# TropComplique/single-shot-detector

Hardware: AMD Instinct MI355X
Metric: images/sec at 896x640, MobileNet-v1 RetinaNet (whole hot path incl. decode + per-class NMS) (higher is better)
Workload: dtype f32

## Files before the change

include/ssd_hip.h:

```cpp
#ifndef SSD_HIP_H
#define SSD_HIP_H

#include <stddef.h>
#include <stdint.h>

#ifdef __cplusplus
extern "C" {
#endif

#define SSD_OK 0
#define SSD_ERR_INVALID (-1)
#define SSD_ERR_HIP (-2)
#define SSD_ERR_STATE (-3)
#define SSD_ERR_WEIGHT (-4)

#define SSD_ACT_NONE 0
#define SSD_ACT_RELU 1
#define SSD_ACT_RELU6 2

#define SSD_BACKBONE_MOBILENET 0
#define SSD_BACKBONE_SHUFFLENET 1

#define SSD_PRECISION_F32 0
#define SSD_PRECISION_F16X3 1
// ... 33 lines not shown
int ssd_forward_records(ssd_handle *h, const uint8_t *images_dev, int32_t B, int32_t H, int32_t W,
                        void *records_dev, void *stream);
int ssd_forward_host(ssd_handle *h, const uint8_t *images_host, int32_t B, int32_t H, int32_t W,
                     void *records, void *stream);

int ssd_network_shape(ssd_handle *h, int32_t height, int32_t width, int32_t *net_hw_out );
int ssd_forward_mixed(ssd_handle *h, const uint8_t *images_dev, int32_t B, const int32_t *hw_host, const int64_t *offsets_host,
                      void *records_dev, void *stream);
int ssd_forward_mixed_host(ssd_handle *h, const uint8_t *const *frames_host, int32_t B, const int32_t *hw_host, void *records,
                           void *stream);

int ssd_detect_host(ssd_handle *h, const uint8_t *image_host, int32_t H, int32_t W, float score_threshold,
                    void *record, float *boxes_out, int32_t *labels_out, float *scores_out, int32_t capacity,
                    int32_t *n_out, void *stream);

int ssd_get_tensor(ssd_handle *h, const char *name, float *host_dst, int64_t capacity_floats,
                   int32_t *dims_out);

int ssd_get_tensor_dev(ssd_handle *h, const char *name, float *dst_dev, int64_t capacity_floats,
                       int32_t *dims_out, void *stream);

int ssd_plan_cache_stats(ssd_handle *h, int64_t *out8);
int ssd_plan_cache_clear(ssd_handle *h);

int ssd_profile_enable(ssd_handle *h, int32_t on);
int ssd_profile_read(ssd_handle *h, int32_t cls, double *total_ms, int64_t *launches,
                     double *flops, double *bytes);
int ssd_profile_reset(ssd_handle *h);


int32_t ssd_num_anchors(int32_t H, int32_t W);
int ssd_anchors(int32_t H, int32_t W, float *anchors_host );
int64_t ssd_anchors_ex(int32_t H, int32_t W, int32_t n_levels, const int32_t *strides, const double *scales,
                       int32_t n_mult, const double *multipliers, int32_t n_ratios, const double *ratios,
                       float *anchors_host, int64_t capacity_rows);

int ssd_conv2d(const float *in_dev, int32_t B, int32_t H, int32_t W, int32_t Cin,
               const float *w_host , int32_t k, int32_t Cout,
               int32_t stride, int32_t pad_beg, int32_t OH, int32_t OW,
               const float *bn_mean_host, const float *bn_sf_host, const float *bn_beta_host,
               const float *bias_host, const float *up_dev, int32_t act, float *out_dev,
               void *stream);

int ssd_conv2d_f16x3(const float *in_dev, int32_t B, int32_t H, int32_t W, int32_t Cin,
                     const float *w_host , int32_t k, int32_t Cout,
                     int32_t stride, int32_t pad_beg, int32_t OH, int32_t OW,
// ... 241 lines not shown
```

single-shot-detector_amd/_lib.py:

```python
import ctypes
import os
import subprocess

_HERE = os.path.dirname(os.path.abspath(__file__))
_CSRC = os.path.join(_HERE, "csrc")
_SOURCES = ["abi.hip", "weights.hip", "plan.hip", "stages.hip", "igemm.hip", "igemm_lat.hip", "igemm16.hip", "logit_screen.hip", "dwpw_stream.hip", "sn_pw.hip", "front.hip",
            "elementwise.hip", "postprocess.hip", "loss.hip", "augment.hip", "update.hip", "train_head.hip", "wgrad.hip", "train_backbone.hip", "train_shufflenet.hip",
            "train_first_f32.hip", "train_norms.hip", "train_hist.hip", "train_reduce.hip"]
_LIB_PATH = os.path.join(_CSRC, "libssd_hip.so")
_DIAG_PATH = os.path.join(_CSRC, "libssd_hip_diag.so")
_lib = None
_diag = False

HIPCC_FLAGS = ["--offload-arch=gfx950", "-O3", "-ffp-contract=off", "-fPIC", "-shared", "-std=c++17"]


class SsdError(RuntimeError):
    """A non-zero return code from libssd_hip.so (message from ssd_last_error())."""


def lib_path():
    return _LIB_PATH


# ... 106 lines not shown
class SsdBnLevel(ctypes.Structure):
    _fields_ = [("rows", ctypes.c_int64)] + [(n, ctypes.c_void_p) for n in (
        "x", "dy", "out", "gamma", "beta", "moving_mean", "moving_variance", "mean", "var", "invstd", "dgamma", "dbeta")]


SIGNATURES = {
    "ssd_create": (ctypes.c_int, [ctypes.POINTER(SsdConfig), ctypes.POINTER(_vp)]),
    "ssd_destroy": (None, [_vp]),
    "ssd_last_error": (ctypes.c_char_p, []),
    "ssd_load_weight": (ctypes.c_int, [_vp, ctypes.c_char_p, _f, ctypes.POINTER(ctypes.c_int64), _i]),
    "ssd_finalize": (ctypes.c_int, [_vp]),
    "ssd_forward": (ctypes.c_int, [_vp, _vp, _i, _i, _i, _vp, _vp, _vp, _vp, _vp]),
    "ssd_record_words": (ctypes.c_int32, [_vp]),
    "ssd_forward_records": (ctypes.c_int, [_vp, _vp, _i, _i, _i, _vp, _vp]),
    "ssd_forward_host": (ctypes.c_int, [_vp, _vp, _i, _i, _i, _vp, _vp]),
    "ssd_network_shape": (ctypes.c_int, [_vp, _i, _i, _i32p]),
    "ssd_forward_mixed": (ctypes.c_int, [_vp, _vp, _i, _i32p, ctypes.POINTER(ctypes.c_int64), _vp, _vp]),
    "ssd_forward_mixed_host": (ctypes.c_int, [_vp, ctypes.POINTER(ctypes.c_void_p), _i, _i32p, _vp, _vp]),
    "ssd_detect_host": (ctypes.c_int, [_vp, _vp, _i, _i, ctypes.c_float, _vp, _vp, _vp, _vp, _i, _i32p, _vp]),
    "ssd_get_tensor": (ctypes.c_int, [_vp, ctypes.c_char_p, _f, ctypes.c_int64, _i32p]),
    "ssd_get_tensor_dev": (ctypes.c_int, [_vp, ctypes.c_char_p, _vp, ctypes.c_int64, _i32p, _vp]),
    "ssd_plan_cache_stats": (ctypes.c_int, [_vp, ctypes.POINTER(ctypes.c_int64)]),
    "ssd_plan_cache_clear": (ctypes.c_int, [_vp]),
    "ssd_profile_enable": (ctypes.c_int, [_vp, _i]),
    "ssd_profile_read": (ctypes.c_int, [_vp, _i, ctypes.POINTER(ctypes.c_double),
                                        ctypes.POINTER(ctypes.c_int64),
                                        ctypes.POINTER(ctypes.c_double),
                                        ctypes.POINTER(ctypes.c_double)]),
    "ssd_profile_reset": (ctypes.c_int, [_vp]),
    "ssd_num_anchors": (ctypes.c_int32, [_i, _i]),
    "ssd_anchors": (ctypes.c_int, [_i, _i, _f]),
    "ssd_anchors_ex": (ctypes.c_int64, [_i, _i, _i, _i32p, ctypes.POINTER(ctypes.c_double), _i, ctypes.POINTER(ctypes.c_double),
                                        _i, ctypes.POINTER(ctypes.c_double), _f, ctypes.c_int64]),
    "ssd_conv2d": (ctypes.c_int, [_vp, _i, _i, _i, _i, _f, _i, _i, _i, _i, _i, _i, _f, _f, _f, _f,
                                  _vp, _i, _vp, _vp]),
    "ssd_conv2d_f16x3": (ctypes.c_int, [_vp, _i, _i, _i, _i, _f, _i, _i, _i, _i, _i, _i, _f, _f, _f, _f,
                                        _vp, _i, _vp, _vp]),
    "ssd_set_option": (ctypes.c_int, [_vp, ctypes.c_char_p, _i]),
    "ssd_get_option": (ctypes.c_int, [_vp, ctypes.c_char_p, _i32p]),
    "ssd_set_precision": (ctypes.c_int, [_vp, _i]),
    "ssd_get_precision": (ctypes.c_int, [_vp]),
    "ssd_status": (ctypes.c_int, [_vp, _i32p]),
    "ssd_depthwise3x3": (ctypes.c_int, [_vp, _i, _i, _i, _i, _f, _i, _i, _i, _i, _f, _f, _f, _i,
                                        _vp, _vp]),
    "ssd_dw_pw": (ctypes.c_int, [_vp, _i, _i, _i, _i, _f, _i, _f, _f, _f, _i, _f, _i, _f, _f, _f, _i, _vp, _vp]),
    "ssd_first_conv": (ctypes.c_int, [_vp, _i, _i, _i, _f, _i, _f, _f, _f, _i, _vp, _vp]),
# ... 119 lines not shown
```

single-shot-detector_amd/csrc/abi.hip:

```cpp
#include "host.h"

#include <algorithm>
#include <cmath>
#include <cstdio>
#include <cstring>

static thread_local std::string g_err;
int ssd_fail(int code, const std::string &msg) { g_err = msg; return code; }
extern "C" const char *ssd_last_error(void) { return g_err.c_str(); }

static Options g_opts;
static std::mutex g_opts_mu;
static const char *const OPT_NAMES[OPT_COUNT] = {"streams", "h2d_chunks", "front_fuse", "fuse_dw", "backbone_split", "event_fence", "plan_cache_mb",
                                                 "igemm_tile", "igemm16", "igemm_96", "igemm_lat", "igemm_deep64", "lateral_split", "fpn_group", "fpn_p7_group",
                                                 "fpn_early_lat", "nsub", "nms_fast_max", "first_conv_px", "debug_sync", "logits_screen",
                                                 "hist_scheme"};
int ssd_opt_index(const char *key)
{
    for (int i = 0; i < OPT_COUNT; ++i)
        if (key && !strcmp(key, OPT_NAMES[i])) return i;
    return -1;
}
int ssd_opt(const ssd_handle *h, int key, int dflt)
{
    if (h && h->opts.v[key] != SSD_OPT_UNSET) return h->opts.v[key];
    const int g = g_opts.v[key];
    return g != SSD_OPT_UNSET ? g : dflt;
}
unsigned ssd_sync_event_flags(const ssd_handle *h)
{
    return hipEventDisableTiming | (ssd_opt(h, OPT_EVENT_FENCE, 0) ? 0u : (unsigned)hipEventDisableSystemFence);
}
int nms_fast_max(const ssd_handle *h)
{
    const int v = ssd_opt(h, OPT_NMS_FAST_MAX, -1);
    return v < 0 ? 0 : (v == 0 ? -1 : v);
}

// ... 492 lines not shown
        else HIPCHK(hipMemcpyAsync(dst_dev + done, r.dev, (size_t)rows * r.C * sizeof(float), hipMemcpyDeviceToDevice, (hipStream_t)stream));
        done += rows * r.C;
        Btot += r.B;
        dims[1] = r.H; dims[2] = r.W; dims[3] = r.C;
    }
    dims[0] = Btot;
    return SSD_OK;
}

extern "C" int ssd_plan_cache_stats(ssd_handle *h, int64_t *out)
{
    if (!h || !out) return ssd_fail(SSD_ERR_INVALID, "ssd_plan_cache_stats: null argument");
    std::lock_guard<std::mutex> g(h->mu);
    HIPCHK(hipSetDevice(h->cfg.device));
    size_t total = 0;
    for (const PlanSet *ps : h->cache) total += ps->bytes;
    out[0] = (int64_t)h->cache.size();
    out[1] = (int64_t)total;
    out[2] = (int64_t)plan_cache_limit_bytes(h);
    out[3] = h->cache_hits; out[4] = h->cache_misses; out[5] = h->cache_evictions;
    out[6] = h->cur ? h->cur->key.netH : 0;
    out[7] = h->cur ? h->cur->key.netW : 0;
    return SSD_OK;
}

extern "C" int ssd_plan_cache_clear(ssd_handle *h)
{
    if (!h) return ssd_fail(SSD_ERR_INVALID, "ssd_plan_cache_clear: null handle");
    std::lock_guard<std::mutex> g(h->mu);
    HIPCHK(hipSetDevice(h->cfg.device));
    HIPCHK(hipDeviceSynchronize());
    h->cache_evictions += (long long)h->cache.size();
    free_plans(h);
    h->n_rec_ok = 0;
    return SSD_OK;
}

extern "C" int ssd_profile_enable(ssd_handle *h, int32_t on)
{
    if (!h) return ssd_fail(SSD_ERR_INVALID, "null handle");
    std::lock_guard<std::mutex> g(h->mu);
    h->profiling = on != 0;
    return SSD_OK;
}

static int drain_events(ssd_handle *h)
// ... 59 lines not shown
```

single-shot-detector_amd/csrc/host.h:

```cpp
#pragma once
#include "../../include/ssd_hip.h"
#include "ssd_internal.h"

#include <climits>
#include <functional>
#include <map>
#include <mutex>
#include <string>
#include <vector>

int ssd_fail(int code, const std::string &msg);
#define HIPCHK(expr)                                                                         \
    do {                                                                                     \
        hipError_t e_ = (expr);                                                              \
        if (e_ != hipSuccess)                                                                \
            return ssd_fail(SSD_ERR_HIP, std::string(#expr) + ": " + hipGetErrorString(e_)); \
    } while (0)
#define SSDCHK(expr)                                                                         \
    do {                                                                                     \
        int r_ = (expr);                                                                     \
        if (r_ != SSD_OK) return r_;                                                         \
    } while (0)

enum SsdOpt {
    OPT_STREAMS = 0,
    OPT_H2D_CHUNKS,
    OPT_FRONT_FUSE,
    OPT_FUSE_DW,
    OPT_BACKBONE_SPLIT,
    OPT_EVENT_FENCE,
    OPT_PLAN_CACHE_MB,
    OPT_IGEMM_TILE,
    OPT_IGEMM16,
    OPT_IGEMM_96,
    OPT_IGEMM_LAT,
    OPT_IGEMM_DEEP64,
    OPT_LATERAL_SPLIT,
    OPT_FPN_GROUP,
    OPT_FPN_P7_GROUP,
    OPT_FPN_EARLY_LAT,
    OPT_NSUB,
    OPT_NMS_FAST_MAX,
    OPT_FIRST_CONV_PX,
    OPT_DEBUG_SYNC,
    OPT_LOGITS_SCREEN,
    OPT_HIST_SCHEME,
    OPT_COUNT
};
#define SSD_OPT_UNSET INT_MIN
struct Options { int v[OPT_COUNT]; Options() { for (int &x : v) x = SSD_OPT_UNSET; } };
int ssd_opt(const struct ssd_handle *h, int key, int dflt);
int ssd_opt_index(const char *key);
unsigned ssd_sync_event_flags(const struct ssd_handle *h);

struct Tensor {
    std::vector<int64_t> shape;
    std::vector<float> data;
};

struct DevPool {
    std::vector<void *> ptrs;
    size_t bytes = 0;
    int alloc(void **out, size_t nbytes)
    {
        HIPCHK(hipMalloc(out, nbytes + 256));
        ptrs.push_back(*out);
        bytes += nbytes + 256;
        return SSD_OK;
// ... 106 lines not shown
int nms_fast_max(const struct ssd_handle *h);

struct ResizeDims { int nh, nw, ph, pw; float box_scaler[4]; };
ResizeDims resize_dims(int height, int width, int min_dimension, int divisor);
extern const int A_STRIDES[5];
extern const int MB_STRIDE[13];

struct Retained { const float *dev; int B, H, W, C, Cp; bool permuted; int fmt = 0;
                  int split = 0;  };

struct EvPair { hipEvent_t a, b; int cls; int fwd; };

struct Plan {
    int B = 0, img0 = 0, N = 0;
    DevPool pool;
    std::vector<Op> ops;
    PostArgs post;
    std::map<std::string, Retained> retained;
    hipStream_t s_aux = nullptr;
    hipStream_t s_bb[2] = {nullptr, nullptr};
    hipEvent_t ev_join = nullptr, ev_begin = nullptr;
    bool need_begin = false;
    bool screened = false, logits_whole = true;
    Op logits_dense;
};

struct SrcGeom { int srcH = 0, srcW = 0, nh = 0, nw = 0; float box_scaler[4] = {1, 1, 1, 1}; };

struct MixedCall { MixedGeom geom; float scaler[SSD_MIXED_MAX][2]; };

struct PlanKey {
    int B = 0, netH = 0, netW = 0, ident = 0, nsub = 0;
    bool operator==(const PlanKey &o) const { return B == o.B && netH == o.netH && netW == o.netW && ident == o.ident && nsub == o.nsub; }
};
struct PlanSet {
    PlanKey key;
    std::vector<Plan *> plans;
    size_t bytes = 0;
    unsigned long long last_use = 0;
};

struct ssd_handle {
    ssd_config cfg;
    std::mutex mu;
    Options opts;
    std::map<std::string, Tensor> vars;
// ... 52 lines not shown
```

single-shot-detector_amd/csrc/logit_screen.hip:

```cpp
#include "ssd_internal.h"
#include <type_traits>

typedef float v16f __attribute__((ext_vector_type(16)));
typedef float v4f __attribute__((ext_vector_type(4)));
typedef unsigned v4u __attribute__((ext_vector_type(4)));
typedef _Float16 v8h __attribute__((ext_vector_type(8)));
typedef short v2s __attribute__((ext_vector_type(2)));
typedef __attribute__((address_space(3))) void *lds_ptr_t;

#define SCREEN_STAGE_BYTES ((256 + 128) * 128)
#define SCREEN_STAGES 3

__device__ __forceinline__ unsigned f16_up_bits(float x)
{
    if (!(x >= 0.0f)) return 0x7e00u;
    if (x == 0.0f) return 0u;
    const _Float16 h = (_Float16)x;
    unsigned b = (unsigned)__builtin_bit_cast(unsigned short, h);
    if ((float)h < x) b += 1u;
    return b < 0x0400u ? 0x0400u : b;
}

__global__ __launch_bounds__(256) void logit_convert_kernel(const float *__restrict__ x, unsigned short *__restrict__ x16, long long n8)
{
// ... 3 lines not shown
        o[0] = f16_up_bits(a[0]) | (f16_up_bits(a[1]) << 16);
        o[1] = f16_up_bits(a[2]) | (f16_up_bits(a[3]) << 16);
        o[2] = f16_up_bits(b[0]) | (f16_up_bits(b[1]) << 16);
        o[3] = f16_up_bits(b[2]) | (f16_up_bits(b[3]) << 16);
        *(v4u *)(x16 + i * 8) = o;
    }
}

__device__ __forceinline__ ScreenLevel screen_level_of_tile(const ScreenArgs &a, int tile_m)
{
    ScreenLevel L = a.lv[0];
#pragma unroll
    for (int i = 1; i < SCREEN_MAX_LEVELS; ++i)
        if (i < a.nlevels && tile_m >= a.lv[i].tile_begin) L = a.lv[i];
    return L;
}
__device__ __forceinline__ ScreenLevel screen_level_of_row(const ScreenArgs &a, int r)
{
    ScreenLevel L = a.lv[0];
#pragma unroll
    for (int i = 1; i < SCREEN_MAX_LEVELS; ++i)
        if (i < a.nlevels && r >= a.lv[i].row_begin) L = a.lv[i];
    return L;
}

__device__ __forceinline__ v8h screen_operand(v4u f, unsigned sgn)
{
    v4u o;
#pragma unroll
    for (int d = 0; d < 4; ++d) {
        const v2s h = __builtin_bit_cast(v2s, f[d] ^ sgn);
        o[d] = __builtin_bit_cast(unsigned, __builtin_elementwise_max(h, v2s{0, 0}));
    }
    return __builtin_bit_cast(v8h, o);
}

__global__ __launch_bounds__(256, 1) void logit_screen_kernel(const ScreenArgs a)
{
    constexpr int BM = 256;
    constexpr int A_BYTES = BM * 128;
    constexpr int STAGE = SCREEN_STAGE_BYTES;
    constexpr int NSTAGE = SCREEN_STAGES;
    extern __shared__ __attribute__((aligned(16))) unsigned char lds[];

    const int tid = threadIdx.x, lane = tid & 63;
    const int wave = __builtin_amdgcn_readfirstlane(tid >> 6);
// ... 158 lines not shown
        for (int j = 0; j < 4; ++j)
#pragma unroll
            for (int r = 0; r < 16; ++r) mine[(r * 4 + j) * 64 + lane] = acc[i][j][r];
        __syncthreads();
        const int rbase = m0 + wave_m * 128 + i * 32;
#pragma unroll 1
        for (int r = wave_n * 8; r < wave_n * 8 + 8; ++r) {
            const int rowl = rbase + (r & 3) + 8 * (r >> 2) + 4 * (lane >> 5);
#pragma unroll
            for (int j = 0; j < 4; ++j) {
                const float Pv = Pp[(r * 4 + j) * 64 + lane], Nv = Np[(r * 4 + j) * 64 + lane];
                const float t1 = Pv * 1.001953125f, t2 = Nv * 0.998046875f;
                const float U = ((t1 - t2) + cst[j]) + 3.814697265625e-06f * ((Pv + Nv) + __builtin_fabsf(cst[j]));
                const bool flag = colok[j] && rowl < M && !(U < lo);
                const unsigned long long mask = __ballot(flag);
                if (mask != 0ull && lane < 8) {
                    const unsigned byte = (unsigned)(mask >> (8 * lane)) & 0xffu;
                    const int row = rbase + (r & 3) + 8 * (r >> 2) + 4 * (lane >> 2);
                    const int col8 = tile_n * 128 + j * 32 + (lane & 3) * 8;
                    if (byte && row < M && col8 < a.Cout) {
                        const int b = row / P, p = row - b * P;
                        const unsigned oct = (unsigned)((out_off + (long long)b * bstride + (long long)p * rstride + col8) >> 3);
                        atomicOr(a.bits + (oct >> 5), 1u << (oct & 31));
                    }
                }
            }
        }
        __syncthreads();
    };
    pass(std::integral_constant<int, 0>{});
    pass(std::integral_constant<int, 1>{});
    pass(std::integral_constant<int, 2>{});
    pass(std::integral_constant<int, 3>{});
}

__global__ __launch_bounds__(256) void logit_compact_kernel(const ScreenArgs a, long long nwords)
{
    __shared__ int lcnt[SCREEN_MAX_OCT], lbase[SCREEN_MAX_OCT];
    __shared__ unsigned short slot[256 * 32];
    const int NO = a.Cout >> 3;
    const unsigned NC = (unsigned)a.out_bstride;
    for (long long w0 = (long long)blockIdx.x * 256; w0 < nwords; w0 += (long long)gridDim.x * 256) {
        const long long w = w0 + threadIdx.x;
        const unsigned bits = w < nwords ? a.bits[w] : 0u;
        if (!__syncthreads_or(bits != 0u)) continue;
        if ((int)threadIdx.x < NO) lcnt[threadIdx.x] = 0;
// ... 83 lines not shown
                    if (!ok) { v0 = v4f{0.f, 0.f, 0.f, 0.f}; v1 = v0; }
                    acc = __builtin_fmaf(v0[0], wp[(k8 + 0) * 8], acc);
                    acc = __builtin_fmaf(v1[0], wp[(k8 + 4) * 8], acc);
                    acc = __builtin_fmaf(v0[1], wp[(k8 + 1) * 8], acc);
                    acc = __builtin_fmaf(v1[1], wp[(k8 + 5) * 8], acc);
                    acc = __builtin_fmaf(v0[2], wp[(k8 + 2) * 8], acc);
                    acc = __builtin_fmaf(v1[2], wp[(k8 + 6) * 8], acc);
                    acc = __builtin_fmaf(v0[3], wp[(k8 + 3) * 8], acc);
                    acc = __builtin_fmaf(v1[3], wp[(k8 + 7) * 8], acc);
                }
            }
            a.logits[L.out_off + (long long)b * a.out_bstride + (long long)p * a.out_rstride + o * 8 + c] = acc + bias;
        }
    }
}

static bool screen_args_ok(const ScreenArgs &a)
{
    if (!a.x || !a.x16 || !a.w16 || !a.wt || !a.bias || !a.cst || !a.logits || !a.bits || !a.counts || !a.lists) return false;
    if (a.Cin % 64 != 0 || a.Cin < 64 || a.Cout % 8 != 0 || a.Cout < 8 || a.Cout > 8 * SCREEN_MAX_OCT || a.Cout > a.CoutPad) return false;
    if (a.NT != (a.Cout + 127) / 128 || a.nlevels < 1 || a.nlevels > SCREEN_MAX_LEVELS) return false;
    if ((long long)9 * a.NT * 128 * a.Cin * 2 >= (1LL << 31) || (long long)9 * a.Cin * 8 * 4 > 160 * 1024 / 2) return false;
    if (a.out_rstride != a.Cout || a.out_bstride <= 0 || (a.out_bstride & 7) || (long long)a.B * a.out_bstride * 4 >= (1LL << 31)) return false;
    long long rows = 0, tiles = 0, outs = 0;
    for (int i = 0; i < a.nlevels; ++i) {
        const ScreenLevel &L = a.lv[i];
        if (L.P != L.H * L.W || L.M != a.B * L.P || L.P < 1 || L.row_begin != rows || L.tile_begin != tiles) return false;
        if ((long long)a.B * L.P * a.Cin * 4 >= (1LL << 31) || L.out_off != outs || (L.out_off & 7)) return false;
        rows += L.M;
        tiles += (L.M + 255) / 256;
        outs += (long long)L.P * a.out_rstride;
    }
    return rows == a.rows_total && tiles == a.tiles_m && outs == a.out_bstride && tiles * a.NT <= 0x7fffffffLL;
}

hipError_t launch_logit_convert(const ScreenArgs &a, hipStream_t s)
{
    if (!screen_args_ok(a) || a.x_elems <= 0 || (a.x_elems & 7)) return hipErrorInvalidValue;
    const long long n8 = a.x_elems / 8;
    const long long nblk = (n8 + 255) / 256;
    hipLaunchKernelGGL(logit_convert_kernel, dim3((unsigned)(nblk < 8192 ? nblk : 8192)), dim3(256), 0, s, a.x, a.x16, n8);
    return hipGetLastError();
}

hipError_t launch_logit_screen(const ScreenArgs &a, hipStream_t s)
{
    if (!screen_args_ok(a)) return hipErrorInvalidValue;
    constexpr int lds_bytes = SCREEN_STAGES * SCREEN_STAGE_BYTES;
    static std::atomic<unsigned> attr_done{0};
    hipError_t e = ssd_allow_lds((const void *)logit_screen_kernel, lds_bytes, attr_done);
    if (e != hipSuccess) return e;
    hipLaunchKernelGGL(logit_screen_kernel, dim3((unsigned)(a.tiles_m * a.NT)), dim3(256), lds_bytes, s, a);
    return hipGetLastError();
}

hipError_t launch_logit_fill(const ScreenArgs &a, hipStream_t s)
{
    if (!screen_args_ok(a)) return hipErrorInvalidValue;
    const long long nwords = ((long long)a.B * a.out_bstride / 8 + 31) / 32;
    const long long cblk = (nwords + 255) / 256;
    hipLaunchKernelGGL(logit_compact_kernel, dim3((unsigned)(cblk < 4096 ? cblk : 4096)), dim3(256), 0, s, a, nwords);
    hipError_t e = hipGetLastError();
    if (e != hipSuccess) return e;
    const int lds_bytes = 9 * a.Cin * 8 * 4;
    static std::atomic<unsigned> attr_done{0};
    e = ssd_allow_lds((const void *)logit_fill_kernel, lds_bytes, attr_done);
    if (e != hipSuccess) return e;
    long long maxchunks = ((long long)a.rows_total + FILL_CHUNK - 1) / FILL_CHUNK * (a.Cout / 8);
    static std::atomic<int> cu_count{0};
    int cus = cu_count.load(std::memory_order_relaxed);
// ... 12 lines not shown
```

single-shot-detector_amd/csrc/plan.hip:

```cpp
#include "host.h"
#include <chrono>

#include <algorithm>
#include <cmath>
#include <cstdio>
#include <cstring>

Op make_conv_op(const ssd_handle *h, const ConvW &cw, const ConvIO &io, int B, int stride, int pad, int act,
                const std::vector<LevelDesc> &lv, bool dense, unsigned *scan_bits, float scan_lo, bool *scan_marked)
{
    const float *in = io.in, *res = io.res;
    float *out = io.out, *out2 = io.out2;
    const int in_fmt = io.in_fmt, out_fmt = io.out_fmt, res_fmt = io.res_fmt;
    int *flags = io.flags;
    IgemmArgs a;
    memset(&a, 0, sizeof(a));
    a.in = in; a.wt = in_fmt ? cw.wt16 : cw.wt; a.out = out; a.out2 = out2;
    a.wt_lat = in_fmt ? nullptr : cw.wlat;
    a.in_fmt = in_fmt; a.out_fmt = out_fmt; a.res_fmt = res ? res_fmt : 0;
    a.acc_scale = in_fmt ? cw.scale16 : 1.0f;
    a.flags = flags;
    a.mean = cw.mean; a.sf = cw.sf; a.beta = cw.beta; a.bias = cw.bias; a.res = res;
    a.B = B; a.Cin = cw.CinP; a.Cout = cw.CoutP; a.CoutPad = cw.CoutPad; a.taps = cw.taps;
    a.stride = stride; a.pad = pad; a.act = act;
// ... 738 lines not shown
{
    ssd_handle *h = b.h;
    Plan &pl = b.pl;
    const Pyr &py = f.py;
    const int B = b.B, C = h->cfg.num_classes, A = 6;
    long long N = 0, aoff[5];
    for (int l = 0; l < 5; ++l) { aoff[l] = N; N += (long long)py.h[l] * py.w[l] * A; }
    pl.N = (int)N;
    float *logits, *codes;
    SSDCHK(b.falloc(&logits, (long long)B * N * C));
    SSDCHK(b.falloc(&codes, (long long)B * N * 4));
    std::vector<float> anc((size_t)N * 4);
    SSDCHK(ssd_anchors(b.H, b.W, anc.data()));
    float *anc_dev;
    SSDCHK(pl.pool.upload(&anc_dev, anc));
    long long rows_total = 0;
    for (int l = 0; l < 5; ++l) rows_total += (long long)B * py.h[l] * py.w[l];
    const int scr_opt = ssd_opt(h, OPT_LOGITS_SCREEN, -1);
    const bool screen = !b.X16 && scr_opt != 0 && ((long long)N * C) % 8 == 0 && (A * C) % 8 == 0 && A * C <= 8 * SCREEN_MAX_OCT &&
                        h->final_[1].wscr && h->final_[1].scst && h->final_[1].CinP == 256 && h->final_[1].CoutP == A * C &&
                        (scr_opt > 0 || rows_total >= SSD_SCREEN_MIN_ROWS);
    float *TAB[2][2];
    unsigned char *keys_home = nullptr;
    {
        const size_t slot = scratch_slot((size_t)py.total * sizeof(float));
        unsigned char *tb = bb.scratch;
        size_t tb_bytes = bb.scratch_bytes;
        if (!bb.scratch || 4 * slot > bb.scratch_bytes) {
            SSDCHK(pl.pool.alloc((void **)&tb, 4 * slot));
            tb_bytes = 4 * slot;
        }
        for (int t = 0; t < 2; ++t)
            for (int k = 0; k < 2; ++k) TAB[t][k] = (float *)(tb + (size_t)(2 * t + k) * slot);
        if (post_keys_bytes(B, (int)N, C) <= tb_bytes && !screen) keys_home = tb;
    }
    void *ws;
    const size_t wsb = post_workspace_bytes(B, (int)N, C, h->cfg.max_boxes_per_class, keys_home == nullptr);
    SSDCHK(pl.pool.alloc(&ws, wsb));
    PostArgs &p = pl.post;
    memset(&p, 0, sizeof(p));
    p.logits = logits; p.codes = codes; p.anchors = anc_dev;
    p.B = B; p.N = (int)N; p.C = C;
    p.score_thr = h->cfg.score_threshold; p.iou_thr = h->cfg.iou_threshold;
    p.max_per_class = h->cfg.max_boxes_per_class;
    p.fast_max = nms_fast_max(h);
    for (int k = 0; k < 4; ++k) p.box_scaler[k] = 1.0f;
    post_carve(p, ws, keys_home);
    HIPCHK(hipMemset(p.scan_bits, 0, post_scan_bitmap_bytes(B, (int)N, C)));
// ... 15 lines not shown
        const bool can_mark = t == 1 && ((long long)N * C) % 8 == 0 && (6 * C) % 8 == 0;
        std::vector<LevelDesc> lv;
        for (int l = 0; l < 5; ++l) {
            LevelDesc d = dense_level(py.h[l], py.w[l], py.h[l], py.w[l], 0, py.off[l]);
            d.out_off = aoff[l] * per;
            d.out_bstride = N * per;
            d.out_rstride = A * per;
            d.param_off = 0;
            lv.push_back(d);
        }
        ConvIO io = b.io16(in, t == 0 ? codes : logits);
        io.out_fmt = 0;
        bool marked = false;
        Op fop = make_conv_op(h, h->final_[t], io, B, 1, 1, SSD_ACT_NONE, lv, false, can_mark ? p.scan_bits : nullptr,
                              conservative_logit_bound(h->cfg.score_threshold), &marked);
        if (t == 1 && screen) {
            pl.logits_dense = make_conv_op(h, h->final_[t], io, B, 1, 1, SSD_ACT_NONE, lv, false);
            pl.screened = true;
            ScreenArgs sa;
            memset(&sa, 0, sizeof(sa));
            const ConvW &fc = h->final_[t];
            sa.x = in;
            sa.x16 = (unsigned short *)TAB[1][cur];
            sa.w16 = fc.wscr; sa.wt = fc.wt; sa.bias = fc.bias; sa.cst = fc.scst;
            sa.logits = logits; sa.bits = p.scan_bits;
            SSDCHK(pl.pool.alloc((void **)&sa.counts, SCREEN_MAX_OCT * sizeof(int)));
            SSDCHK(pl.pool.alloc((void **)&sa.lists, (size_t)(A * C / 8) * (size_t)rows_total * sizeof(int)));
            HIPCHK(hipMemset(sa.counts, 0, SCREEN_MAX_OCT * sizeof(int)));
            sa.lo = conservative_logit_bound(h->cfg.score_threshold);
            sa.B = B; sa.Cin = fc.CinP; sa.Cout = fc.CoutP; sa.CoutPad = fc.CoutPad; sa.NT = (fc.CoutP + 127) / 128;
            sa.nlevels = 5;
            sa.out_rstride = A * C; sa.out_bstride = N * C;
            sa.x_elems = py.total;
            int rows = 0, tiles = 0;
            for (int l = 0; l < 5; ++l) {
                ScreenLevel &L = sa.lv[l];
                L.H = py.h[l]; L.W = py.w[l]; L.P = L.H * L.W; L.M = B * L.P;
                L.row_begin = rows; L.tile_begin = tiles;
                L.in_off = py.off[l]; L.out_off = aoff[l] * C;
                rows += L.M;
                tiles += (L.M + 255) / 256;
            }
            sa.rows_total = rows; sa.tiles_m = tiles;
            Op o;
            o.cls = 4; o.flops = 0;
            if (scr_opt == 2) {
                const size_t lbytes = (size_t)B * N * C * sizeof(float);
                o.bytes = (double)lbytes;
                o.run = [logits, lbytes](hipStream_t s) { return hipMemsetAsync(logits, 0xff, lbytes, s); };
                tower_ops[t].push_back(o);
            }
            o.bytes = (double)py.total * 6.0;
            o.run = [sa](hipStream_t s) { return launch_logit_convert(sa, s); };
            tower_ops[t].push_back(o);
            o.bytes = (double)py.total * 2.0 + (double)fc.taps * sa.NT * 128 * fc.CinP * 2.0;
            o.run = [sa](hipStream_t s) { return launch_logit_screen(sa, s); };
            tower_ops[t].push_back(o);
            o.bytes = (double)B * N * C / 64.0;
            o.run = [sa](hipStream_t s) { return launch_logit_fill(sa, s); };
            tower_ops[t].push_back(o);
            continue;
        }
        if (t == 1) all_marked = all_marked && marked;
        tower_ops[t].push_back(fop);
    }
    p.scan_fused = all_marked ? 1 : 0;
    for (size_t i = 0; i < std::max(tower_ops[0].size(), tower_ops[1].size()); ++i)
        for (int t = 1; t >= 0; --t) {
            if (i >= tower_ops[t].size()) continue;
            std::vector<int> deps;
            if (i == 0) { deps.push_back(t == 0 ? f.id_p4 : f.id_p3); deps.push_back(f.id_p7); }
            b.push(tower_ops[t][i], t, deps);
        }
    pl.retained["encoded_boxes"] = Retained{codes, B, 1, (int)N, 4, 4, false};
    pl.retained["class_predictions"] = Retained{logits, B, 1, (int)N, C, C, false};
    pl.retained["class_logits_filled"] = Retained{logits, B, 1, (int)N, C, C, false};
    return SSD_OK;
}
// ... 280 lines not shown
```

single-shot-detector_amd/csrc/ssd_internal.h:

```cpp
#pragma once
#include <hip/hip_runtime.h>
#include <stdint.h>

__host__ __device__ static inline int ssd_phys_of_logical(int l) { int o = l & ~7, r = l & 7; return o + ((r & 1) ? 4 + (r >> 1) : (r >> 1)); }
__host__ __device__ static inline int ssd_logical_of_phys(int p) { int o = p & ~7, r = p & 7; return o + (r < 4 ? 2 * r : 2 * (r - 4) + 1); }

#define SSD_MAX_LEVELS 10

#include <atomic>
static inline hipError_t ssd_allow_lds(const void *fn, int bytes, std::atomic<unsigned> &done)
{
    int dev = 0;
    hipError_t e = hipGetDevice(&dev);
    if (e != hipSuccess) return e;
    if (dev >= 0 && dev < 32 && ((done.load(std::memory_order_relaxed) >> dev) & 1u)) return hipSuccess;
    e = hipFuncSetAttribute(fn, hipFuncAttributeMaxDynamicSharedMemorySize, bytes);
    if (e == hipSuccess && dev >= 0 && dev < 32) done.fetch_or(1u << dev, std::memory_order_relaxed);
    return e;
}

struct UDiv { unsigned mag; int sh; };
static inline UDiv ssd_udiv_make(unsigned d)
{
    UDiv u;
// ... 61 lines not shown
                    IGEMM_LAT_W2_1x1 = 24, IGEMM_LAT_W4_1x1 = 25, IGEMM_LAT_W4_2x1 = 26, IGEMM_LAT_W4_1x2 = 27,
                    IGEMM_LAT_1x1_IL = 28, IGEMM_LAT_1x1_D8 = 29, IGEMM_LAT_1x1_D16 = 30, IGEMM_LAT_1x1_NM = 31, IGEMM_LAT_1x1_D8_NM = 32 };
#ifdef SSD_DIAG
static inline bool igemm_is_lat(int tile) { return tile >= IGEMM_LAT_1x1 && tile <= 36; }
#else
static inline bool igemm_is_lat(int tile) { return (tile >= IGEMM_LAT_1x1 && tile <= IGEMM_LAT_W4_1x2) || tile == IGEMM_LAT_1x1_D16; }
#endif
int igemm_lat_bm(int tile);
int igemm_lat_bn(int tile);
bool igemm_lat_n_major(int tile);
bool igemm_lat_supports(const IgemmArgs &a);
hipError_t launch_igemm_lat(int tile, const IgemmArgs &a, int total_tiles_m, hipStream_t s);
#define IGEMM16_TILE 100
hipError_t launch_igemm16(const IgemmArgs &a, int total_tiles_m, hipStream_t s);

#define SCREEN_MAX_LEVELS 5
#define SCREEN_MAX_OCT 128
struct ScreenLevel {
    int H, W, P, M;
    int row_begin;
    int tile_begin;
    long long in_off;
    long long out_off;
};
struct ScreenArgs {
    const float *x;
    unsigned short *x16;
    const unsigned short *w16;
    const float *wt;
    const float *bias;
    const float *cst;
    float *logits;
    unsigned *bits;
    int *counts;
    int *lists;
    float lo;
    int B, Cin, Cout, CoutPad, NT;
    int nlevels, tiles_m, rows_total;
    int out_rstride;
    long long out_bstride;
    long long x_elems;
    ScreenLevel lv[SCREEN_MAX_LEVELS];
};
hipError_t launch_logit_convert(const ScreenArgs &a, hipStream_t s);
hipError_t launch_logit_screen(const ScreenArgs &a, hipStream_t s);
hipError_t launch_logit_fill(const ScreenArgs &a, hipStream_t s);

struct DwPwSArgs {
    const float *in;
    const float *dwpack;
    const float *wt;
    const float *mean, *sf, *beta;
    float *out;
    int out_rs;
    int B, H, W, K, OH, OW, Cout, wt_rows;
    int pad;
    int dact, act;
    int tiles_y, tiles_x, m_tiles, n_tiles;
    int out_bytes;
    long long *ts;
    int abl;
// ... 117 lines not shown
```

single-shot-detector_amd/ssd.py:

```python
import ctypes
import threading

import numpy as np

from . import _lib
from ._lib import SsdConfig, SsdLossConfig, check, lib

ACT = {None: 0, "none": 0, "relu": 1, "relu6": 2}


def _torch():
    import torch
    if not torch.cuda.is_available():
        raise RuntimeError("single-shot-detector_amd needs an AMD GPU (HIP device): there is "
                           "no CPU path")
    return torch


def _stream(torch):
    return ctypes.c_void_p(torch.cuda.current_stream().cuda_stream)


def _ptr(t):
    return ctypes.c_void_p(t.data_ptr())
# ... 717 lines not shown
            e["cmp"].record(s_c)
            with torch.cuda.stream(s_out):
                s_out.wait_event(e["cmp"])
                oslot["pin_out"].copy_(oslot["block"], non_blocking=True)
                e["d2h"].record(s_out)
            if pending is not None:
                yield collect(pending)
            pending = (oslot, e)
            k += 1
        if pending is not None:
            yield collect(pending)

    def plan_cache_stats(self):
        v = (ctypes.c_int64 * 8)()
        with self.lock:
            check(lib().ssd_plan_cache_stats(self._h, v))
        return {"plans": v[0], "arena_bytes": v[1], "budget_bytes": v[2], "hits": v[3], "misses": v[4], "evictions": v[5],
                "last_network_shape": [v[6], v[7]]}

    def plan_cache_clear(self):
        with self.lock:
            check(lib().ssd_plan_cache_clear(self._h))

    def get_tensor(self, name):
        dims = (ctypes.c_int32 * 4)()
        cap = 1 << 20
        while True:
            buf = np.empty((cap,), np.float32)
            with self.lock:
                rc = lib().ssd_get_tensor(self._h, name.encode(),
                                          buf.ctypes.data_as(ctypes.POINTER(ctypes.c_float)), cap, dims)
            if rc != 0 and b"too small" in (lib().ssd_last_error() or b"") and cap < (1 << 34):
                cap *= 8
                continue
            check(rc)
            n = dims[0] * dims[1] * dims[2] * dims[3]
            return buf[:n].reshape(dims[0], dims[1], dims[2], dims[3]).copy()

    def get_tensor_dev(self, name, shape):
        torch = _torch()
        out = torch.empty(tuple(shape), dtype=torch.float32, device="cuda:%d" % self.device)
        dims = (ctypes.c_int32 * 4)()
        with self.lock:
            check(lib().ssd_get_tensor_dev(self._h, name.encode(), _ptr(out), out.numel(), dims,
                                           _stream(torch)))
        return out
# ... 117 lines not shown
```

Before: 879.0.

## Add halo-padded f16 input layout and LDS-staged halo kernel for logit screen

```diff
diff --git a/include/ssd_hip.h b/include/ssd_hip.h
--- a/include/ssd_hip.h
+++ b/include/ssd_hip.h
@@ -79,6 +79,8 @@
 
 int ssd_plan_cache_stats(ssd_handle *h, int64_t *out8);
 int ssd_plan_cache_clear(ssd_handle *h);
+int ssd_screen_form(ssd_handle *h);
+int64_t ssd_screen_halo_lds_bytes(int32_t nlevels, const int32_t *widths);
 
 int ssd_profile_enable(ssd_handle *h, int32_t on);
 int ssd_profile_read(ssd_handle *h, int32_t cls, double *total_ms, int64_t *launches,
diff --git a/single-shot-detector_amd/_lib.py b/single-shot-detector_amd/_lib.py
--- a/single-shot-detector_amd/_lib.py
+++ b/single-shot-detector_amd/_lib.py
@@ -152,6 +152,8 @@
     "ssd_get_tensor_dev": (ctypes.c_int, [_vp, ctypes.c_char_p, _vp, ctypes.c_int64, _i32p, _vp]),
     "ssd_plan_cache_stats": (ctypes.c_int, [_vp, ctypes.POINTER(ctypes.c_int64)]),
     "ssd_plan_cache_clear": (ctypes.c_int, [_vp]),
+    "ssd_screen_form": (ctypes.c_int, [_vp]),
+    "ssd_screen_halo_lds_bytes": (ctypes.c_int64, [_i, _i32p]),
     "ssd_profile_enable": (ctypes.c_int, [_vp, _i]),
     "ssd_profile_read": (ctypes.c_int, [_vp, _i, ctypes.POINTER(ctypes.c_double),
                                         ctypes.POINTER(ctypes.c_int64),
diff --git a/single-shot-detector_amd/csrc/abi.hip b/single-shot-detector_amd/csrc/abi.hip
--- a/single-shot-detector_amd/csrc/abi.hip
+++ b/single-shot-detector_amd/csrc/abi.hip
@@ -13,7 +13,7 @@
 static std::mutex g_opts_mu;
 static const char *const OPT_NAMES[OPT_COUNT] = {"streams", "h2d_chunks", "front_fuse", "fuse_dw", "backbone_split", "event_fence", "plan_cache_mb",
                                                  "igemm_tile", "igemm16", "igemm_96", "igemm_lat", "igemm_deep64", "lateral_split", "fpn_group", "fpn_p7_group",
-                                                 "fpn_early_lat", "nsub", "nms_fast_max", "first_conv_px", "debug_sync", "logits_screen",
+                                                 "fpn_early_lat", "nsub", "nms_fast_max", "first_conv_px", "debug_sync", "logits_screen", "screen_halo",
                                                  "hist_scheme"};
 int ssd_opt_index(const char *key)
 {
@@ -552,6 +552,23 @@
     out[6] = h->cur ? h->cur->key.netH : 0;
     out[7] = h->cur ? h->cur->key.netW : 0;
     return SSD_OK;
+}
+
+extern "C" int ssd_screen_form(ssd_handle *h)
+{
+    if (!h) return ssd_fail(SSD_ERR_INVALID, "ssd_screen_form: null handle");
+    std::lock_guard<std::mutex> g(h->mu);
+    if (!h->cur || h->cur->plans.empty()) return ssd_fail(SSD_ERR_STATE, "ssd_screen_form before ssd_forward");
+    const Plan *pl = h->cur->plans[0];
+    return !pl->screened ? 0 : (pl->screen_halo ? 2 : 1);
+}
+
+extern "C" int64_t ssd_screen_halo_lds_bytes(int32_t nlevels, const int32_t *widths)
+{
+    if (!widths || nlevels < 1 || nlevels > SCREEN_MAX_LEVELS) return 0;
+    int w[SCREEN_MAX_LEVELS];
+    for (int i = 0; i < nlevels; ++i) w[i] = widths[i];
+    return screen_halo_lds_bytes(nlevels, w);
 }
 
 extern "C" int ssd_plan_cache_clear(ssd_handle *h)
diff --git a/single-shot-detector_amd/csrc/host.h b/single-shot-detector_amd/csrc/host.h
--- a/single-shot-detector_amd/csrc/host.h
+++ b/single-shot-detector_amd/csrc/host.h
@@ -44,6 +44,7 @@
     OPT_FIRST_CONV_PX,
     OPT_DEBUG_SYNC,
     OPT_LOGITS_SCREEN,
+    OPT_SCREEN_HALO,
     OPT_HIST_SCHEME,
     OPT_COUNT
 };
@@ -196,6 +197,7 @@
     hipEvent_t ev_join = nullptr, ev_begin = nullptr;
     bool need_begin = false;
     bool screened = false, logits_whole = true;
+    bool screen_halo = false;
     Op logits_dense;
 };
 
diff --git a/single-shot-detector_amd/csrc/logit_screen.hip b/single-shot-detector_amd/csrc/logit_screen.hip
--- a/single-shot-detector_amd/csrc/logit_screen.hip
+++ b/single-shot-detector_amd/csrc/logit_screen.hip
@@ -49,6 +49,33 @@
     for (int i = 1; i < SCREEN_MAX_LEVELS; ++i)
         if (i < a.nlevels && r >= a.lv[i].row_begin) L = a.lv[i];
     return L;
+}
+
+__global__ __launch_bounds__(256) void logit_convert_halo_kernel(const ScreenArgs a)
+{
+    const unsigned KC = (unsigned)a.Cin >> 6;
+    const long long n = (long long)a.prows_total * KC * 8;
+    for (long long i = (long long)blockIdx.x * 256 + threadIdx.x; i < n; i += (long long)gridDim.x * 256) {
+        const unsigned chunk = (unsigned)i & 7u, j = (unsigned)(i >> 3);
+        const unsigned gq = j / KC, kc = j - gq * KC;
+        ScreenLevel L = a.lv[0];
+#pragma unroll
+        for (int l = 1; l < SCREEN_MAX_LEVELS; ++l)
+            if (l < a.nlevels && (int)gq >= a.lv[l].prow_begin) L = a.lv[l];
+        const unsigned q = gq - (unsigned)L.prow_begin;
+        const unsigned b = q / (unsigned)L.Pp, rem = q - b * (unsigned)L.Pp;
+        const unsigned yp = rem / (unsigned)L.Wp, xp = rem - yp * (unsigned)L.Wp;
+        v4u o = v4u{0u, 0u, 0u, 0u};
+        if (yp >= 1u && yp <= (unsigned)L.H && xp >= 1u && xp <= (unsigned)L.W) {
+            const float *src = a.x + L.in_off + ((long long)b * L.P + (long long)(yp - 1u) * L.W + (xp - 1u)) * a.Cin + kc * 64u + chunk * 8u;
+            const v4f u = *(const v4f *)src, v = *(const v4f *)(src + 4);
+            o[0] = f16_up_bits(u[0]) | (f16_up_bits(u[1]) << 16);
+            o[1] = f16_up_bits(u[2]) | (f16_up_bits(u[3]) << 16);
+            o[2] = f16_up_bits(v[0]) | (f16_up_bits(v[1]) << 16);
+            o[3] = f16_up_bits(v[2]) | (f16_up_bits(v[3]) << 16);
+        }
+        *(v4u *)(a.x16 + L.plane_off + ((long long)kc * L.Mp + q) * 64 + chunk * 8u) = o;
+    }
 }
 
 __device__ __forceinline__ v8h screen_operand(v4u f, unsigned sgn)
@@ -253,6 +280,239 @@
                         const int b = row / P, p = row - b * P;
                         const unsigned oct = (unsigned)((out_off + (long long)b * bstride + (long long)p * rstride + col8) >> 3);
                         atomicOr(a.bits + (oct >> 5), 1u << (oct & 31));
+                    }
+                }
+            }
+        }
+        __syncthreads();
+    };
+    pass(std::integral_constant<int, 0>{});
+    pass(std::integral_constant<int, 1>{});
+    pass(std::integral_constant<int, 2>{});
+    pass(std::integral_constant<int, 3>{});
+}
+
+#define SCREEN_HALO_B_BYTES (128 * 128)
+#define SCREEN_HALO_FIXED_BYTES (2 * SCREEN_HALO_B_BYTES + 1024)
+
+long long screen_halo_lds_bytes(int nlevels, const int *widths)
+{
+    int wmax = 0;
+    for (int i = 0; i < nlevels; ++i) {
+        if (widths[i] < 1) return 0;
+        wmax = widths[i] > wmax ? widths[i] : wmax;
+    }
+    if (nlevels < 1 || wmax > 4096) return 0;
+    const int G = wmax + 3;
+    const long long np = (256 + 2 * G + 7) / 8;
+    const long long bytes = 2 * np * 1024 + SCREEN_HALO_FIXED_BYTES;
+    return np <= 64 && bytes <= SCREEN_HALO_LDS_MAX ? bytes : 0;
+}
+
+__global__ __launch_bounds__(256, 1) void logit_screen_halo_kernel(const ScreenArgs a)
+{
+    constexpr int BM = 256;
+    constexpr int B_BYTES = SCREEN_HALO_B_BYTES;
+    extern __shared__ __attribute__((aligned(16))) unsigned char lds[];
+
+    const int tid = threadIdx.x, lane = tid & 63;
+    const int wave = __builtin_amdgcn_readfirstlane(tid >> 6);
+    const int wave_m = wave >> 1, wave_n = wave & 1;
+    const unsigned sgn = wave_n ? 0x80008000u : 0u;
+    int swz;
+    {
+        const int nblk = gridDim.x, bid = blockIdx.x;
+        const int q = nblk >> 3, r = nblk & 7, xcd = bid & 7;
+        swz = (xcd < r ? xcd * (q + 1) : r * (q + 1) + (xcd - r) * q) + (bid >> 3);
+    }
+    const int tile_n = swz % a.NT;
+    const int tile_m = swz / a.NT;
+    const ScreenLevel L = screen_level_of_tile(a, tile_m);
+    const int H = L.H, W = L.W, Wp = L.Wp, Pp = L.Pp, Mp = L.Mp;
+    const int G = Wp + 1;
+    const int NP = (BM + 2 * G + 7) >> 3;
+    const int Cin = a.Cin;
+    const int q0 = (tile_m - L.tile_begin) * BM;
+    const int ABUF = (a.halo_lds - SCREEN_HALO_FIXED_BYTES) >> 1;
+    unsigned char *const bst = lds + 2 * ABUF;
+    unsigned char *const dump = bst + 2 * B_BYTES;
+
+    const __amdgpu_buffer_rsrc_t arsrc = __builtin_amdgcn_make_buffer_rsrc(
+        (void *)(a.x16 + L.plane_off), 0, (int)((long long)Mp * Cin * 2), 0x00020000);
+    const __amdgpu_buffer_rsrc_t brsrc = __builtin_amdgcn_make_buffer_rsrc(
+        (void *)a.w16, 0, (int)((long long)9 * a.NT * 128 * Cin * 2), 0x00020000);
+    constexpr unsigned OOB = 0x80000000u;
+
+    int boff[4];
+#pragma unroll
+    for (int u = 0; u < 4; ++u) {
+        const int row = wave * 32 + u * 8 + (lane >> 3);
+        const int chunk = (lane & 7) ^ ((row >> 1) & 7);
+        boff[u] = (tile_n * 128 + row) * Cin * 2 + chunk * 16;
+    }
+    const int b_tapstride = a.NT * 128 * Cin * 2;
+    const int KC = Cin >> 6;
+    const int KS = 9 * KC;
+    int dtap = 0, dkc = 0;
+    auto dma_b = [&](unsigned char *stage) {
+        const bool live = dkc < KC;
+        unsigned char *bbuf = stage + wave * 32 * 128;
+        const int bso = live ? dtap * b_tapstride + dkc * 128 : 0;
+#pragma unroll
+        for (int u = 0; u < 4; ++u)
+            __builtin_amdgcn_raw_ptr_buffer_load_lds(brsrc, (lds_ptr_t)(bbuf + u * 1024), 16, live ? boff[u] : (int)OOB, bso, 0, 0);
+        if (++dtap == 9) { dtap = 0; ++dkc; }
+    };
+    auto dma_a = [&](int kc2, int slot, unsigned char *abuf) {
+        const int p = wave + 4 * slot;
+        const int rr = p * 8 + (lane >> 3);
+        const int q = q0 - G + rr;
+        const bool ok = (kc2 < KC) & (p < NP) & ((unsigned)q < (unsigned)Mp);
+        const int chunk = (lane & 7) ^ ((rr >> 1) & 7);
+        const unsigned off = ok ? (unsigned)(((kc2 * Mp + q) << 7) + (chunk << 4)) : OOB;
+        unsigned char *dst = p < NP ? abuf + p * 1024 : dump;
+        __builtin_amdgcn_raw_ptr_buffer_load_lds(arsrc, (lds_ptr_t)dst, 16, (int)off, 0, 0, 0);
+    };
+    auto afrag = [&](int kc2, int tap2, int (&ao)[4]) {
+        const int ky = tap2 / 3, kx = tap2 - 3 * ky;
+        const int rr0 = G + (ky - 1) * Wp + (kx - 1) + wave_m * 128 + (lane & 31);
+        const int key = (rr0 >> 1) & 7;
+        const int base = (kc2 & 1) * ABUF + rr0 * 128;
+#pragma unroll
+        for (int s = 0; s < 4; ++s) ao[s] = base + (((2 * s + (lane >> 5)) ^ key) << 4);
+    };
+    int roff[4];
+#pragma unroll
+    for (int s = 0; s < 4; ++s) {
+        const int chunk = 2 * s + (lane >> 5);
+        roff[s] = (lane & 31) * 128 + ((chunk ^ (((lane & 31) >> 1) & 7)) << 4);
+    }
+    auto rd = [&](const int (&ao)[4], const unsigned char *bb, int s, v4f (&fa)[4], v4u (&fb)[4]) {
+#pragma unroll
+        for (int i = 0; i < 4; ++i) fa[i] = *(const v4f *)(lds + ao[s] + i * 4096);
+#pragma unroll
+        for (int j = 0; j < 4; ++j) fb[j] = *(const v4u *)(bb + j * 4096 + roff[s]);
+    };
+    v16f acc[4][4];
+#pragma unroll
+    for (int i = 0; i < 4; ++i)
+#pragma unroll
+        for (int j = 0; j < 4; ++j)
+#pragma unroll
+            for (int r = 0; r < 16; ++r) acc[i][j][r] = 0.0f;
+    auto mf = [&](const v4f (&fa)[4], const v4u (&fb)[4]) {
+#pragma unroll
+        for (int j = 0; j < 4; ++j) {
+            const v8h bj = screen_operand(fb[j], sgn);
+#pragma unroll
+            for (int i = 0; i < 4; ++i)
+                acc[i][j] = __builtin_amdgcn_mfma_f32_32x32x16_f16(__builtin_bit_cast(v8h, fa[i]), bj, acc[i][j], 0, 0, 0);
+        }
+    };
+    auto sched = [&](bool with_dma) {
+#pragma unroll
+        for (int i = 0; i < 16; ++i) {
+            __builtin_amdgcn_sched_group_barrier(0x008, 1, 0);
+            if (i < 8) __builtin_amdgcn_sched_group_barrier(0x100, 1, 0);
+            if (with_dma && i >= 4 && i < 10) __builtin_amdgcn_sched_group_barrier(0x020, 1, 0);
+            if (with_dma) __builtin_amdgcn_sched_group_barrier(0x006, 8, 0);
+            else __builtin_amdgcn_sched_group_barrier(0x006, 6, 0);
+        }
+        __builtin_amdgcn_sched_barrier(0);
+    };
+
+#pragma unroll
+    for (int slot = 0; slot < 16; ++slot) dma_a(0, slot, lds);
+    dma_b(bst);
+    dma_b(bst + B_BYTES);
+    asm volatile("s_waitcnt vmcnt(0) lgkmcnt(0)" ::: "memory");
+    __builtin_amdgcn_s_barrier();
+    __builtin_amdgcn_sched_barrier(0);
+
+    v4f fa0[4], fa1[4];
+    v4u fb0[4], fb1[4];
+    int ao[4], an[4];
+    int tap = 0, kc = 0;
+    unsigned char *bcur = bst, *bnxt = bst + B_BYTES;
+    afrag(0, 0, ao);
+    rd(ao, bcur, 0, fa0, fb0);
+#pragma unroll 1
+    for (int ks = 0; ks < KS; ++ks) {
+        rd(ao, bcur, 1, fa1, fb1);
+        mf(fa0, fb0);
+        sched(false);
+        rd(ao, bcur, 2, fa0, fb0);
+        mf(fa1, fb1);
+        sched(false);
+        int ntap = tap + 1, nkc = kc;
+        if (ntap == 9) { ntap = 0; ++nkc; }
+        afrag(nkc, ntap, an);
+        rd(ao, bcur, 3, fa1, fb1);
+        mf(fa0, fb0);
+        sched(false);
+        asm volatile("s_waitcnt vmcnt(0) lgkmcnt(0)" ::: "memory");
+        __builtin_amdgcn_s_barrier();
+        __builtin_amdgcn_sched_barrier(0);
+        rd(an, bnxt, 0, fa0, fb0);
+        dma_b(bcur);
+        unsigned char *const anext = lds + ((kc + 1) & 1) * ABUF;
+        dma_a(kc + 1, 2 * tap, anext);
+        dma_a(kc + 1, 2 * tap + 1, anext);
+        mf(fa1, fb1);
+        sched(true);
+        unsigned char *const t = bcur;
+        bcur = bnxt; bnxt = t;
+        tap = ntap; kc = nkc;
+#pragma unroll
+        for (int s = 0; s < 4; ++s) ao[s] = an[s];
+    }
+
+    asm volatile("s_waitcnt vmcnt(0) lgkmcnt(0)" ::: "memory");
+    __syncthreads();
+    if (blockIdx.x == 0 && tid < (a.Cout >> 3)) a.counts[tid] = 0;
+    float *mine = (float *)lds + wave * 4096;
+    const float *Ps = (const float *)lds + (wave_m * 2) * 4096, *Ns = Ps + 4096;
+    float cst[4];
+    bool colok[4];
+#pragma unroll
+    for (int j = 0; j < 4; ++j) {
+        const int col = tile_n * 128 + j * 32 + (lane & 31);
+        colok[j] = col < a.Cout;
+        cst[j] = colok[j] ? a.cst[col] : 0.0f;
+    }
+    const float lo = a.lo;
+    const int rstride = a.out_rstride;
+    const long long bstride = a.out_bstride, out_off = L.out_off;
+    auto pass = [&](auto itag) __attribute__((always_inline)) {
+        constexpr int i = decltype(itag)::value;
+#pragma unroll
+        for (int j = 0; j < 4; ++j)
+#pragma unroll
+            for (int r = 0; r < 16; ++r) mine[(r * 4 + j) * 64 + lane] = acc[i][j][r];
+        __syncthreads();
+        const int rbase = q0 + wave_m * 128 + i * 32;
+#pragma unroll 1
+        for (int r = wave_n * 8; r < wave_n * 8 + 8; ++r) {
+            const int rowl = rbase + (r & 3) + 8 * (r >> 2) + 4 * (lane >> 5);
+#pragma unroll
+            for (int j = 0; j < 4; ++j) {
+                const float Pv = Ps[(r * 4 + j) * 64 + lane], Nv = Ns[(r * 4 + j) * 64 + lane];
+                const float t1 = Pv * 1.001953125f, t2 = Nv * 0.998046875f;
+                const float U = ((t1 - t2) + cst[j]) + 3.814697265625e-06f * ((Pv + Nv) + __builtin_fabsf(cst[j]));
+                const bool flag = colok[j] && rowl < Mp && !(U < lo);
+                const unsigned long long mask = __ballot(flag);
+                if (mask != 0ull && lane < 8) {
+                    const unsigned byte = (unsigned)(mask >> (8 * lane)) & 0xffu;
+                    const int row = rbase + (r & 3) + 8 * (r >> 2) + 4 * (lane >> 2);
+                    const int col8 = tile_n * 128 + j * 32 + (lane & 3) * 8;
+                    if (byte && row < Mp && col8 < a.Cout) {
+                        const int b = row / Pp, rem = row - b * Pp;
+                        const int yp = rem / Wp, xp = rem - yp * Wp;
+                        if (yp >= 1 && yp <= H && xp >= 1 && xp <= W) {
+                            const int p = (yp - 1) * W + (xp - 1);
+                            const unsigned oct = (unsigned)((out_off + (long long)b * bstride + (long long)p * rstride + col8) >> 3);
+                            atomicOr(a.bits + (oct >> 5), 1u << (oct & 31));
+                        }
                     }
                 }
             }
@@ -382,21 +642,38 @@
     if (a.NT != (a.Cout + 127) / 128 || a.nlevels < 1 || a.nlevels > SCREEN_MAX_LEVELS) return false;
     if ((long long)9 * a.NT * 128 * a.Cin * 2 >= (1LL << 31) || (long long)9 * a.Cin * 8 * 4 > 160 * 1024 / 2) return false;
     if (a.out_rstride != a.Cout || a.out_bstride <= 0 || (a.out_bstride & 7) || (long long)a.B * a.out_bstride * 4 >= (1LL << 31)) return false;
-    long long rows = 0, tiles = 0, outs = 0;
+    long long rows = 0, tiles = 0, outs = 0, prows = 0, plane = 0;
+    int widths[SCREEN_MAX_LEVELS];
     for (int i = 0; i < a.nlevels; ++i) {
         const ScreenLevel &L = a.lv[i];
         if (L.P != L.H * L.W || L.M != a.B * L.P || L.P < 1 || L.row_begin != rows || L.tile_begin != tiles) return false;
         if ((long long)a.B * L.P * a.Cin * 4 >= (1LL << 31) || L.out_off != outs || (L.out_off & 7)) return false;
+        if (a.halo) {
+            if (L.Wp != L.W + 2 || (long long)L.Pp != (long long)(L.H + 2) * L.Wp || (long long)L.Mp != (long long)a.B * L.Pp) return false;
+            if ((long long)a.B * L.Pp * a.Cin * 2 >= (1LL << 31) || L.prow_begin != prows || L.plane_off != plane) return false;
+            prows += L.Mp;
+            plane += (long long)L.Mp * a.Cin;
+            widths[i] = L.W;
+        }
         rows += L.M;
-        tiles += (L.M + 255) / 256;
+        tiles += ((a.halo ? L.Mp : L.M) + 255) / 256;
         outs += (long long)L.P * a.out_rstride;
     }
+    if (a.halo) {
+        if (a.halo != 1 || prows != a.prows_total || prows * (a.Cin >> 6) * 8 >= (1LL << 31) || plane * 2 > a.x16_bytes) return false;
+        if (a.halo_lds <= 0 || a.halo_lds != screen_halo_lds_bytes(a.nlevels, widths)) return false;
+    } else if (a.x_elems * 2 > a.x16_bytes) return false;
     return rows == a.rows_total && tiles == a.tiles_m && outs == a.out_bstride && tiles * a.NT <= 0x7fffffffLL;
 }
 
 hipError_t launch_logit_convert(const ScreenArgs &a, hipStream_t s)
 {
     if (!screen_args_ok(a) || a.x_elems <= 0 || (a.x_elems & 7)) return hipErrorInvalidValue;
+    if (a.halo) {
+        const long long nb = ((long long)a.prows_total * (a.Cin >> 3) + 255) / 256;
+        hipLaunchKernelGGL(logit_convert_halo_kernel, dim3((unsigned)(nb < 8192 ? nb : 8192)), dim3(256), 0, s, a);
+        return hipGetLastError();
+    }
     const long long n8 = a.x_elems / 8;
     const long long nblk = (n8 + 255) / 256;
     hipLaunchKernelGGL(logit_convert_kernel, dim3((unsigned)(nblk < 8192 ? nblk : 8192)), dim3(256), 0, s, a.x, a.x16, n8);
@@ -406,6 +683,13 @@
 hipError_t launch_logit_screen(const ScreenArgs &a, hipStream_t s)
 {
     if (!screen_args_ok(a)) return hipErrorInvalidValue;
+    if (a.halo) {
+        static std::atomic<unsigned> halo_attr_done{0};
+        hipError_t e = ssd_allow_lds((const void *)logit_screen_halo_kernel, SCREEN_HALO_LDS_MAX, halo_attr_done);
+        if (e != hipSuccess) return e;
+        hipLaunchKernelGGL(logit_screen_halo_kernel, dim3((unsigned)(a.tiles_m * a.NT)), dim3(256), a.halo_lds, s, a);
+        return hipGetLastError();
+    }
     constexpr int lds_bytes = SCREEN_STAGES * SCREEN_STAGE_BYTES;
     static std::atomic<unsigned> attr_done{0};
     hipError_t e = ssd_allow_lds((const void *)logit_screen_kernel, lds_bytes, attr_done);
diff --git a/single-shot-detector_amd/csrc/plan.hip b/single-shot-detector_amd/csrc/plan.hip
--- a/single-shot-detector_amd/csrc/plan.hip
+++ b/single-shot-detector_amd/csrc/plan.hip
@@ -784,8 +784,8 @@
                         (scr_opt > 0 || rows_total >= SSD_SCREEN_MIN_ROWS);
     float *TAB[2][2];
     unsigned char *keys_home = nullptr;
+    const size_t slot = scratch_slot((size_t)py.total * sizeof(float));
     {
-        const size_t slot = scratch_slot((size_t)py.total * sizeof(float));
         unsigned char *tb = bb.scratch;
         size_t tb_bytes = bb.scratch_bytes;
         if (!bb.scratch || 4 * slot > bb.scratch_bytes) {
@@ -847,6 +847,16 @@
             const ConvW &fc = h->final_[t];
             sa.x = in;
             sa.x16 = (unsigned short *)TAB[1][cur];
+            sa.x16_bytes = (long long)slot;
+            int lvw[5];
+            for (int l = 0; l < 5; ++l) lvw[l] = py.w[l];
+            const int halo_opt = ssd_opt(h, OPT_SCREEN_HALO, -1);
+            const long long halo_lds = screen_halo_lds_bytes(5, lvw);
+            if (halo_opt > 0 && halo_lds == 0)
+                return ssd_fail(SSD_ERR_INVALID, "option screen_halo = 1: a level of this shape is too wide for the halo kernel's LDS");
+            sa.halo = halo_opt != 0 && halo_lds > 0 ? 1 : 0;
+            sa.halo_lds = (int)halo_lds;
+            pl.screen_halo = sa.halo != 0;
             sa.w16 = fc.wscr; sa.wt = fc.wt; sa.bias = fc.bias; sa.cst = fc.scst;
             sa.logits = logits; sa.bits = p.scan_bits;
             SSDCHK(pl.pool.alloc((void **)&sa.counts, SCREEN_MAX_OCT * sizeof(int)));
@@ -857,16 +867,24 @@
             sa.nlevels = 5;
             sa.out_rstride = A * C; sa.out_bstride = N * C;
             sa.x_elems = py.total;
-            int rows = 0, tiles = 0;
+            int rows = 0, tiles = 0, prows = 0;
+            long long plane = 0;
             for (int l = 0; l < 5; ++l) {
                 ScreenLevel &L = sa.lv[l];
                 L.H = py.h[l]; L.W = py.w[l]; L.P = L.H * L.W; L.M = B * L.P;
-                L.row_begin = rows; L.tile_begin = tiles;
+                L.Wp = L.W + 2; L.Pp = (L.H + 2) * L.Wp; L.Mp = B * L.Pp;
+                L.row_begin = rows; L.tile_begin = tiles; L.prow_begin = prows; L.plane_off = plane;
                 L.in_off = py.off[l]; L.out_off = aoff[l] * C;
                 rows += L.M;
-                tiles += (L.M + 255) / 256;
+                prows += L.Mp;
+                plane += (long long)L.Mp * fc.CinP;
+                tiles += ((sa.halo ? L.Mp : L.M) + 255) / 256;
             }
-            sa.rows_total = rows; sa.tiles_m = tiles;
+            sa.rows_total = rows; sa.tiles_m = tiles; sa.prows_total = prows;
+            if (sa.halo && plane * 2 > sa.x16_bytes) {
+                SSDCHK(pl.pool.alloc((void **)&sa.x16, (size_t)plane * 2));
+                sa.x16_bytes = plane * 2;
+            }
             Op o;
             o.cls = 4; o.flops = 0;
             if (scr_opt == 2) {
@@ -875,10 +893,10 @@
                 o.run = [logits, lbytes](hipStream_t s) { return hipMemsetAsync(logits, 0xff, lbytes, s); };
                 tower_ops[t].push_back(o);
             }
-            o.bytes = (double)py.total * 6.0;
+            o.bytes = (double)py.total * 4.0 + (sa.halo ? (double)plane : (double)py.total) * 2.0;
             o.run = [sa](hipStream_t s) { return launch_logit_convert(sa, s); };
             tower_ops[t].push_back(o);
-            o.bytes = (double)py.total * 2.0 + (double)fc.taps * sa.NT * 128 * fc.CinP * 2.0;
+            o.bytes = (sa.halo ? (double)plane : (double)py.total) * 2.0 + (double)fc.taps * sa.NT * 128 * fc.CinP * 2.0;
             o.run = [sa](hipStream_t s) { return launch_logit_screen(sa, s); };
             tower_ops[t].push_back(o);
             o.bytes = (double)B * N * C / 64.0;
diff --git a/single-shot-detector_amd/csrc/ssd_internal.h b/single-shot-detector_amd/csrc/ssd_internal.h
--- a/single-shot-detector_amd/csrc/ssd_internal.h
+++ b/single-shot-detector_amd/csrc/ssd_internal.h
@@ -107,7 +107,12 @@
     int tile_begin;
     long long in_off;
     long long out_off;
-};
+    int Wp, Pp, Mp;
+    int prow_begin;
+    long long plane_off;
+};
+#define SCREEN_HALO_LDS_MAX (160 * 1024)
+long long screen_halo_lds_bytes(int nlevels, const int *widths);
 struct ScreenArgs {
     const float *x;
     unsigned short *x16;
@@ -122,6 +127,10 @@
     float lo;
     int B, Cin, Cout, CoutPad, NT;
     int nlevels, tiles_m, rows_total;
+    int halo;
+    int prows_total;
+    int halo_lds;
+    long long x16_bytes;
     int out_rstride;
     long long out_bstride;
     long long x_elems;
diff --git a/single-shot-detector_amd/ssd.py b/single-shot-detector_amd/ssd.py
--- a/single-shot-detector_amd/ssd.py
+++ b/single-shot-detector_amd/ssd.py
@@ -763,6 +763,13 @@
         with self.lock:
             check(lib().ssd_plan_cache_clear(self._h))
 
+    def screen_form(self):
+        with self.lock:
+            rc = lib().ssd_screen_form(self._h)
+        if rc < 0:
+            check(rc)
+        return rc
+
     def get_tensor(self, name):
         dims = (ctypes.c_int32 * 4)()
         cap = 1 << 20
```

Result: no change. 883.1 (median of 6 runs) (+0.5%).
